# Parskatt/RoMa

Hardware: AMD Instinct MI355X
Metric: image-pairs/sec, roma_outdoor 560->864, batch=8 per GPU (higher is better)
Workload: dtype bf16; 1 GPU; roma_outdoor match() 560->864, symmetric, upsample_preds, 8 pairs/GPU/step, seeded synthetic weights + N(0,1) images; precision policy of the reference's bf16 timing script: bfloat16 DINOv2 + float16 autocast for VGG / decoder / refiners (ROMA_MIXED), f32 accumulate; precision_policy=mixed, global_batch=8, streams_per_gpu=2, parallelism=single GPU, outputs_finite=True

## Files before the change

roma_amd/csrc/elementwise.h:

```cpp
#pragma once
#include "common.h"

namespace roma {

int layernorm_launch(const float* x, const float* w, const float* b, void* out, long M, int D, float eps,
                     int dt_out, hipStream_t s);
int layernorm_launch_dt(const void* x, int dt_in, const float* w, const float* b, void* out, long M, int D, float eps,
                        int dt_out, hipStream_t s);

int conv3x3_c3_launch(const float* img, const float* w, const float* bias, void* out, int B, int H, int W,
                      int dt_out, hipStream_t s);

int im2col3x3_c3_launch(const float* img, void* out, int B, int H, int W, int dt_out, hipStream_t s);

int maxpool2x2_launch(const void* in, void* out, int B, int H, int W, int C, int dt, hipStream_t s);

int im2col_patch14_launch(const float* img, void* out, int B, int H, int W, int Kpad, int dt_out, hipStream_t s);

int assemble_tokens_launch(const float* patch, const float* cls, const float* pos, float* tokens, int B, int T,
                           int D, hipStream_t s);

int copy2d_launch(const void* in, long ldi, int dt_in, void* out, long ldo, int dt_out, long rows, int cols,
                  hipStream_t s);

int convert_from_bf16_launch(const void* in, void* out, long n, hipStream_t s);

int rownorm_launch(const void* in, long ld, int dt, float* norms, long M, int C, hipStream_t s);

int gp_basis_launch(const float* w, const float* b, float* Ft, int Dg, int h, int wdt, int npad, hipStream_t s, int copies = 1,
                    long stride = 0);

int transpose_launch(const float* in, float* out, int n, long ld, int batch, hipStream_t s, long stride_in = 0, long stride_out = 0);

int chol_diag_launch(float* A, long ld, long strideA, float* Linv, float* LinvT, int k, int nblk, int batch,
                     hipStream_t s);

int chol_col_launch(float* A, long ld, long strideA, float* LT, long strideLT, int n, int d, float* Linv, float* LinvT, int k,
                    int nblk, int batch, unsigned epoch, int use_leader, hipStream_t s);
int chol_col_restore_launch(float* A, long ld, long strideA, const float* LT, long strideLT, int n, int batch, hipStream_t s);

int pad_identity_launch(float* A, long ld, long strideA, int n, int npad, int batch, hipStream_t s);

int cls_to_flow_launch(const float* logits, long ld, float* flow, float* cert, long M, hipStream_t s);

struct RefinerInputArgs {
  const void* feat = nullptr;
  long ldf = 0;
  const float* flow = nullptr;
  void* d = nullptr;
  long ldd = 0;
  const float* emb_w = nullptr;
  const float* emb_b = nullptr;
  int B = 0, H = 0, W = 0, C = 0, E = 0, Kcorr = 0, nimg = 0, shift = 0;
  float disp_scale = 1.f;
  int dt = 0;
};
int refiner_input_launch(const RefinerInputArgs& a, hipStream_t s);

int dwconv5x5_launch(const void* in, void* out, const float* w, const float* bias, int B, int H, int W, int Cp,
                     int dt, hipStream_t s);
int dwconv5x5_ring_try_launch(const void* in, void* out, const float* w, const float* bias, int B, int H, int W, int Cp, int dt,
                              hipStream_t s);
// ... 23 lines not shown
```

roma_amd/csrc/gp.h:

```cpp
#pragma once
#include "arena.h"
#include "common.h"

namespace roma {

int gp_posterior(const void* pf, long ldf, int act_dt, int B, bool symmetric, int th, int tw, const float* gp_w,
                 const float* gp_b, float* mu, long ld_mu, Arena& arena, hipStream_t st, bool dry);

int cholesky_solve_t(float* A, float* Rt, float* LT, float* Linv, float* LinvT, int n, int d, int batch, hipStream_t st,
                     long strideA = 0, long strideR = 0);

}
```

roma_amd/csrc/gp.hip:

```cpp
#include "gp.h"

#include <atomic>

#include "dry_run.h"
#include "elementwise.h"
#include "gemm.h"
#include "tuning.h"

namespace roma {

int cholesky_solve_t(float* A, float* Rt, float* LT, float* Linv, float* LinvT, int n, int d, int batch, hipStream_t st,
                     long strideA, long strideR) {
  ROMA_REQUIRE(n % 64 == 0 && n > 0 && d % 4 == 0, "cholesky_solve: n must be a multiple of 64, d of 4");
  const int nblk = n / 64;
  const long sA = strideA > 0 ? strideA : (long)n * n, sR = strideR > 0 ? strideR : (long)d * n, sL = (long)nblk * 4096;
  const long sLT = (long)n * n;
  const bool aug_env = tuning(SW_GP_AUG) != 0;
  const bool aug = aug_env && Rt == A + (long)n * n && (batch == 1 || (sA == sR && sA >= (long)(n + d) * n));
  const int extra = aug ? d : 0;
  const bool col = aug && tuning(SW_GP_COL) != 0 && d >= 64 && d % 64 == 0;
  static std::atomic<unsigned> solve_epoch{0};
  const unsigned epoch = col ? ++solve_epoch : 0u;
  const int col_leader = col ? (int)tuning(SW_GP_COL_LEADER) : 0;
  for (int k = 0; k < nblk && col; ++k)
    if (int rc = chol_col_launch(A, n, sA, LT, sLT, n, d, Linv, LinvT, k, nblk, batch, epoch, col_leader, st)) return rc;
  if (col)
    if (int rc = chol_col_restore_launch(A, n, sA, LT, sLT, n, batch, st)) return rc;
  for (int k = 0; k < nblk && !col; ++k) {
    if (int rc = chol_diag_launch(A, n, sA, Linv, LinvT, k, nblk, batch, st)) return rc;
    const int mrem = n - (k + 1) * 64;
    if (mrem + extra <= 0) break;
    GemmArgs g;
    g.A = A + (long)(k + 1) * 64 * n + k * 64; g.lda = n; g.sA = sA;
    g.W = Linv + (long)k * 4096; g.ldw = 64; g.sW = sL;
    g.C = const_cast<float*>(static_cast<const float*>(g.A)); g.ldc = n; g.sC = sA;
// ... 18 lines not shown
    g.W = Linv + (long)k * 4096; g.ldw = 64; g.sW = sL;
    g.C = Rt + k * 64; g.ldc = n; g.sC = sR;
    g.M = d; g.N = 64; g.K = 64; g.batch = batch;
    if (int rc = gemm_launch(g, st)) return rc;
    const int mrem = n - (k + 1) * 64;
    if (mrem <= 0) break;
    GemmArgs u;
    u.A = Rt + k * 64; u.lda = n; u.sA = sR;
    u.W = A + (long)(k + 1) * 64 * n + k * 64; u.ldw = n; u.sW = sA;
    u.C = Rt + (k + 1) * 64; u.ldc = n; u.sC = sR;
    u.res = Rt + (k + 1) * 64; u.ldr = n; u.sR = sR;
    u.alpha = -1.f;
    u.M = d; u.N = mrem; u.K = 64; u.batch = batch;
    if (int rc = gemm_launch(u, st)) return rc;
  }
  const bool bwd_env = tuning(SW_GP_BWD2) != 0;
  if (bwd_env && nblk > 1) {
    GemmArgs m;
    m.A = LT; m.lda = n; m.sA = sLT; m.sA2 = 64;
    m.W = Linv; m.ldw = 64; m.sW = sL; m.sW2 = 4096;
    m.C = LT; m.ldc = n; m.sC = sLT; m.sC2 = 64;
    m.M = n; m.N = 64; m.K = 64; m.batch = batch; m.batch2 = nblk;
    if (int rc = gemm_launch(m, st)) return rc;
    for (int k = nblk - 1; k >= 1; --k) {
      GemmArgs u;
      u.A = Rt + k * 64; u.lda = n; u.sA = sR;
      u.W = LT + k * 64; u.ldw = n; u.sW = sLT;
      u.C = Rt; u.ldc = n; u.sC = sR;
      u.res = Rt; u.ldr = n; u.sR = sR;
      u.alpha = -1.f;
      u.M = d; u.N = k * 64; u.K = 64; u.batch = batch;
      if (int rc = gemm_launch(u, st)) return rc;
    }
    GemmArgs x;
    x.A = Rt; x.lda = n; x.sA = sR; x.sA2 = 64;
    x.W = LinvT; x.ldw = 64; x.sW = sL; x.sW2 = 4096;
    x.C = Rt; x.ldc = n; x.sC = sR; x.sC2 = 64;
    x.M = d; x.N = 64; x.K = 64; x.batch = batch; x.batch2 = nblk;
    return gemm_launch(x, st);
  }
  for (int k = nblk - 1; k >= 0; --k) {
    GemmArgs g;
    g.A = Rt + k * 64; g.lda = n; g.sA = sR;
    g.W = LinvT + (long)k * 4096; g.ldw = 64; g.sW = sL;
    g.C = Rt + k * 64; g.ldc = n; g.sC = sR;
    g.M = d; g.N = 64; g.K = 64; g.batch = batch;
    if (int rc = gemm_launch(g, st)) return rc;
// ... 5 lines not shown
    u.res = Rt; u.ldr = n; u.sR = sR;
    u.alpha = -1.f;
    u.M = d; u.N = k * 64; u.K = 64; u.batch = batch;
    if (int rc = gemm_launch(u, st)) return rc;
  }
  return 0;
}

int gp_posterior(const void* pf, long ldf, int act_dt, int B, bool symmetric, int th, int tw, const float* gp_w,
                 const float* gp_b, float* mu, long ld_mu, Arena& arena, hipStream_t st, bool dry) {
  const size_t esz = act_dt == DT_F32 ? 4 : 2;
  const int nimg = 2 * B, ndp = symmetric ? 2 * B : B, shift = B;
  const int n = th * tw, npad = (int)round_up(n, 64), nblk = npad / 64;
  auto AL = [&](size_t elems, size_t es) { return arena.alloc(elems * es); };
  auto off = [&](const void* p, long elems) -> const void* { return static_cast<const char*>(p) + elems * (long)esz; };
  float* norms = (float*)AL((size_t)nimg * n, 4);
  const long saug = (long)(npad + 512) * npad;
  float* Kyy = (float*)AL((size_t)nimg * saug, 4);
  float* Rt = Kyy + (long)npad * npad;
  float* LT = (float*)AL((size_t)nimg * npad * npad, 4);
  float* Kxy = (float*)AL((size_t)ndp * n * npad, 4);
  float* Linv = (float*)AL((size_t)nimg * nblk * 4096, 4);
  float* LinvT = (float*)AL((size_t)nimg * nblk * 4096, 4);
  if (!dry && arena.overflow) return -5;
  RUN(rownorm_launch(pf, ldf, act_dt, norms, (long)nimg * n, 512, st));
  const int j0 = symmetric ? 0 : B, nj = symmetric ? nimg : B;
  {
    GemmArgs g;
    g.A = off(pf, (long)j0 * n * ldf); g.lda = ldf; g.sA = (long)n * ldf;
    g.W = g.A; g.ldw = ldf; g.sW = g.sA;
    g.C = Kyy + (long)j0 * saug; g.ldc = npad; g.sC = saug;
    g.M = n; g.N = n; g.K = 512; g.batch = nj; g.in_dt = act_dt; g.out_dt = DT_F32; g.mode = EPI_COSK;
    g.nx = norms + (long)j0 * n; g.ny = g.nx; g.sNx = n; g.sNy = n; g.inv_t = 1.0f / 0.2f; g.diag_add = 0.1f;
    RUN(gemm_launch(g, st));
  }
  RUN(pad_identity_launch(Kyy + (long)j0 * saug, npad, saug, n, npad, nj, st));
  if (!dry && npad != n) ROMA_CHECK_HIP(hipMemsetAsync(Kxy, 0, (size_t)ndp * n * npad * 4, st));
  for (int half = 0; half < (symmetric ? 2 : 1); ++half) {
    GemmArgs g;
    const int i0 = half * B, s0 = (i0 + shift) % nimg;
    g.A = off(pf, (long)i0 * n * ldf); g.lda = ldf; g.sA = (long)n * ldf;
    g.W = off(pf, (long)s0 * n * ldf); g.ldw = ldf; g.sW = (long)n * ldf;
    g.C = Kxy + (long)i0 * n * npad; g.ldc = npad; g.sC = (long)n * npad;
    g.M = n; g.N = n; g.K = 512; g.batch = B; g.in_dt = act_dt; g.out_dt = DT_F32; g.mode = EPI_COSK;
    g.nx = norms + (long)i0 * n; g.ny = norms + (long)s0 * n; g.sNx = n; g.sNy = n; g.inv_t = 1.0f / 0.2f;
    RUN(gemm_launch(g, st));
  }
  RUN(gp_basis_launch(gp_w, gp_b, Rt + (long)j0 * saug, 512, th, tw, npad, st, nj, saug));
  RUN(cholesky_solve_t(Kyy + (long)j0 * saug, Rt + (long)j0 * saug, LT + (long)j0 * npad * npad,
                          Linv + (long)j0 * nblk * 4096, LinvT + (long)j0 * nblk * 4096, npad, 512, nj, st, saug, saug));
  for (int half = 0; half < (symmetric ? 2 : 1); ++half) {
    GemmArgs g;
    const int i0 = half * B, s0 = (i0 + shift) % nimg;
    g.A = Kxy + (long)i0 * n * npad; g.lda = npad; g.sA = (long)n * npad;
    g.W = Rt + (long)s0 * saug; g.ldw = npad; g.sW = saug;
    g.C = mu + (long)i0 * n * ld_mu; g.ldc = ld_mu; g.sC = (long)n * ld_mu;
    g.M = n; g.N = 512; g.K = npad; g.batch = B;
    RUN(gemm_launch(g, st));
  }
  return 0;
}
}
```

roma_amd/csrc/local_corr.h:

```cpp
#pragma once
#include "common.h"

namespace roma {

struct LocalCorrArgs {
  const void* f0 = nullptr;
  const void* f1 = nullptr;
  const float* warp = nullptr;
  void* out = nullptr;
  int B = 0, H = 0, W = 0, C = 0;
  int radius = 0;
  int K = 0;
  long ld0 = 0, ld1 = 0, ldo = 0;
  int nimg = 0, f1_shift = 0;
  float scale = 1.f;
  int in_dt = 0, out_dt = 0;
  int nearest = 0;
  int* ws = nullptr;
  long ws_bytes = 0;
  int force_gather = 0;
  int pxmax = 0;
  int bin_ts = 0, bin_nx = 0, bin_ny = 0, ws_bins = 0, ws_qlist = 0;
  int sort_bands = 0;
  long ws_tclass = 0, ws_hist = 0;
};

long local_corr_ws_ints(int B, int H, int W, int radius);

int local_corr_window_launch(const LocalCorrArgs& a, hipStream_t stream);
int local_corr_general_launch(const LocalCorrArgs& a, hipStream_t stream);

}
```

roma_amd/csrc/local_corr.hip:

```cpp
#include "local_corr.h"
#include "tuning.h"
#include <stdio.h>
#include <stdlib.h>
#include <algorithm>
#include "gemm.h"

namespace roma {

template <typename T> struct LcIO;
template <> struct LcIO<float> {
  static constexpr int CE = 4;
  __device__ static inline void ld(const float* p, float* v) {
    f32x4 x = *reinterpret_cast<const f32x4*>(p);
    v[0] = x[0]; v[1] = x[1]; v[2] = x[2]; v[3] = x[3];
  }
};
template <> struct LcIO<bf16_t> {
  static constexpr int CE = 8;
  __device__ static inline void ld(const bf16_t* p, float* v) {
    uint4 u = *reinterpret_cast<const uint4*>(p);
    v[0] = h16_lo(u.x); v[1] = h16_hi(u.x);
    v[2] = h16_lo(u.y); v[3] = h16_hi(u.y);
    v[4] = h16_lo(u.z); v[5] = h16_hi(u.z);
    v[6] = h16_lo(u.w); v[7] = h16_hi(u.w);
// ... 157 lines not shown

template <int R, typename T, typename TOUT, bool MFMA, bool LIST = false>
__global__ __launch_bounds__((LcGeom<R, MFMA>::NTHR), 2) void local_corr_tile_kernel(const LocalCorrArgs a) {
  constexpr int P = 2 * R + 2, KW = 2 * R + 1, K = KW * KW;
  constexpr int NTHR = LcGeom<R, MFMA>::NTHR, NWV = NTHR / 64, NBG = NWV / 2;
  constexpr int NR = (P + NWV - 1) / NWV;
  constexpr int NBW = MFMA ? ((LcGeom<R, MFMA>::PXMAX + 31) / 32 + NBG - 1) / NBG : 1;
  static_assert(!MFMA || sizeof(T) == 2, "the MFMA form takes 16-bit features");
  constexpr int CC = LcDot<T>::CC;
  constexpr int LC_STAGE = LcGeom<R, MFMA>::STAGE, LC_PXMAX = LcGeom<R, MFMA>::PXMAX, NPRE = LcGeom<R, MFMA>::NPRE;
  extern __shared__ __attribute__((aligned(16))) char lds[];
  int* qx0 = reinterpret_cast<int*>(lds + LC_STAGE);
  int* qy0 = qx0 + 64;
  float* qfx = reinterpret_cast<float*>(qy0 + 64);
  float* qfy = qfx + 64;
  int* tinfo = reinterpret_cast<int*>(qfy + 64);
  int* qpx = tinfo + 8;

  const int tid = threadIdx.x, lane = tid & 63, wave = tid >> 6;
  const int tiles_x = (a.W + LC_TQ - 1) / LC_TQ, tiles_y = (a.H + LC_TQ - 1) / LC_TQ;
  const int tpi = tiles_x * tiles_y;
  const long HW = (long)a.H * a.W;
  const int* tlist = a.ws + 4 + a.B * tpi;
  for (int tidx = blockIdx.x; tidx < (LIST ? a.ws[2] : a.ws[1]); tidx += gridDim.x) {
  __syncthreads();
  int b, qin;
  if constexpr (LIST) {
    const int* ql = a.ws + a.ws_qlist + (long)tidx * 64;
    const int g = ql[lane];
    b = __shfl(g, 0) / (int)HW;
    qin = g >= 0 ? g - b * (int)HW : -1;
  } else {
    const int tile = tlist[tidx];
    b = tile / tpi;
    const int trem = tile - b * tpi;
    const int ty = trem / tiles_x, tx = trem - ty * tiles_x;
    const int qy = ty * LC_TQ + (lane >> 3), qx = tx * LC_TQ + (lane & 7);
    qin = (qy < a.H && qx < a.W) ? qy * a.W + qx : -1;
  }

  const bool qvalid = qin >= 0;
  const long qpix = (long)b * HW + (qvalid ? qin : 0);
  int x0 = 0, y0 = 0;
  float fx = 0.f, fy = 0.f;
  if (qvalid) {
    unnormalize_floor(a.warp[qpix * 2 + 0], a.W, x0, fx);
    unnormalize_floor(a.warp[qpix * 2 + 1], a.H, y0, fy);
  }
// ... 498 lines not shown
}
long local_corr_ws_ints(int B, int H, int W, int radius) {
  if (radius != 2 && radius != 3 && radius != 7) return 0;
  const long tiles = (long)B * ((H + LC_TQ - 1) / LC_TQ) * ((W + LC_TQ - 1) / LC_TQ);
  const int ts = lc_bin_ts(radius), P = 2 * radius + 2;
  const long nbins = (long)B * ((W + P) / ts + 1) * ((H + P) / ts + 1);
  return 4 + 2 * tiles + 3 * nbins + 64 * (tiles + nbins) + tiles + lc_sort_bands(B, (H + LC_TQ - 1) / LC_TQ) * nbins;
}

template <int R, typename T, typename TOUT, bool MFMA>
static int launch_tiled(const LocalCorrArgs& a0, hipStream_t stream) {
  LocalCorrArgs a = a0;
  const int tiles = a.B * ((a.H + LC_TQ - 1) / LC_TQ) * ((a.W + LC_TQ - 1) / LC_TQ);
  constexpr int P = 2 * R + 2;
  a.bin_ts = lc_bin_ts(R);
  a.bin_nx = (a.W + P) / a.bin_ts + 1;
  a.bin_ny = (a.H + P) / a.bin_ts + 1;
  const long nbins = (long)a.B * a.bin_nx * a.bin_ny;
  a.ws_bins = 4 + 2 * tiles;
  a.ws_qlist = a.ws_bins + 3 * (int)nbins;
  const int lc_bin = tuning(SW_LC_BIN);
  const bool binned = lc_bin != 0 && (long)a.B * a.H * a.W < (1l << 31) &&
                      (a.bin_ts + P - 1) * (a.bin_ts + P - 1) <= LcGeom<R, MFMA>::PXMAX;
  const bool lds_sort = binned && lc_bin == 1 && a.bin_nx * a.bin_ny <= LC_SORT_MAXBINS && 64 * ((long)tiles + nbins) < (1l << 31);
  a.ws_tclass = a.ws_qlist + 64 * ((long)tiles + nbins);
  a.ws_hist = a.ws_tclass + tiles;
  a.sort_bands = lds_sort ? lc_sort_bands(a.B, (a.H + LC_TQ - 1) / LC_TQ) : 0;
  const size_t need = (size_t)local_corr_ws_ints(a.B, a.H, a.W, R) * sizeof(int);
  bool own_ws = false;
  if (!a.ws) {
    ROMA_CHECK_HIP(hipMallocAsync(reinterpret_cast<void**>(&a.ws), need, stream));
    own_ws = true;
  } else {
    ROMA_REQUIRE((size_t)a.ws_bytes >= need, "local_corr(window): work-list scratch too small");
  }
  a.force_gather = tuning_override(SW_LC_MODE) == 1 ? 1 : 0;
  ROMA_CHECK_HIP(hipMemsetAsync(a.ws, 0, 4 * sizeof(int), stream));
  const size_t lds_tile = (size_t)LcGeom<R, MFMA>::STAGE + 5 * 64 * 4 + 32;
  a.pxmax = LcGeom<R, MFMA>::PXMAX;
  static bool attr_set[64] = {false};
  int dev = 0;
  ROMA_CHECK_HIP(hipGetDevice(&dev));
  if (dev < 0 || dev >= 64 || !attr_set[dev]) {
    ROMA_CHECK_HIP(hipFuncSetAttribute(reinterpret_cast<const void*>(&local_corr_tile_kernel<R, T, TOUT, MFMA>),
                                       hipFuncAttributeMaxDynamicSharedMemorySize, (int)lds_tile));
    if (dev >= 0 && dev < 64) attr_set[dev] = true;
  }
// ... 6 lines not shown
      const dim3 sgrid((unsigned)a.sort_bands, (unsigned)a.B);
      hipLaunchKernelGGL((local_corr_sort_kernel<R, false>), sgrid, dim3(LC_SORT_NTHR), 0, stream, a);
      ROMA_LAUNCH_CHECK();
      hipLaunchKernelGGL(local_corr_bin_scan_kernel, dim3(1), dim3(1024), 0, stream, a);
      ROMA_LAUNCH_CHECK();
      hipLaunchKernelGGL((local_corr_sort_kernel<R, true>), sgrid, dim3(LC_SORT_NTHR), 0, stream, a);
      ROMA_LAUNCH_CHECK();
    } else {
      ROMA_CHECK_HIP(hipMemsetAsync(a.ws + a.ws_bins, 0, (size_t)3 * nbins * sizeof(int), stream));
      ROMA_CHECK_HIP(hipMemsetAsync(a.ws + a.ws_qlist, 0xff, (size_t)64 * (tiles + nbins) * sizeof(int), stream));
      hipLaunchKernelGGL((local_corr_bin_kernel<R, false>), dim3((unsigned)tiles), dim3(64), 0, stream, a);
      ROMA_LAUNCH_CHECK();
      hipLaunchKernelGGL(local_corr_bin_scan_kernel, dim3(1), dim3(1024), 0, stream, a);
      ROMA_LAUNCH_CHECK();
      hipLaunchKernelGGL((local_corr_bin_kernel<R, true>), dim3((unsigned)tiles), dim3(64), 0, stream, a);
      ROMA_LAUNCH_CHECK();
    }
    static bool attr_set_l[64] = {false};
    if (dev < 0 || dev >= 64 || !attr_set_l[dev]) {
      ROMA_CHECK_HIP(hipFuncSetAttribute(reinterpret_cast<const void*>(&local_corr_tile_kernel<R, T, TOUT, MFMA, true>),
                                         hipFuncAttributeMaxDynamicSharedMemorySize, (int)lds_tile));
      if (dev >= 0 && dev < 64) attr_set_l[dev] = true;
    }
    const long max_items = (long)tiles + nbins;
    hipLaunchKernelGGL((local_corr_tile_kernel<R, T, TOUT, MFMA, true>), dim3((unsigned)std::min<long>(max_items, 8192)), dim3(LcGeom<R, MFMA>::NTHR),
                       lds_tile, stream, a);
    ROMA_LAUNCH_CHECK();
  } else {
    hipLaunchKernelGGL((local_corr_list_kernel<R, T, TOUT, 4>), dim3((unsigned)tiles * 16u), dim3(256), (size_t)4 * a.C * sizeof(float),
                       stream, a);
    ROMA_LAUNCH_CHECK();
  }
  if (own_ws) ROMA_CHECK_HIP(hipFreeAsync(a.ws, stream));
  return 0;
}

template <int R>
static int launch_window_r(const LocalCorrArgs& a, hipStream_t stream) {
  const long total = (long)a.B * a.H * a.W;
  dim3 grid((unsigned)((total + 3) / 4));
  size_t lds = (size_t)4 * a.C * sizeof(float);
  const double es_in = a.in_dt == DT_F32 ? 4.0 : 2.0, es_out = a.out_dt == DT_F32 ? 4.0 : 2.0;
  char pname[64];
  snprintf(pname, sizeof pname, "local_corr_window_kernel<%d,%s>", R, a.in_dt == DT_F32 ? "f32" : ROMA_H16_NAME);
  ProfScope ps(pname, (double)total * (2.0 * a.C * es_in + 8.0 + (2.0 * R + 1) * (2.0 * R + 1) * es_out), "byte", stream);
  const int mode = tuning(SW_LC_MODE);
  const int cc = a.in_dt == DT_F32 ? 32 : 64;
// ... 55 lines not shown
```

roma_amd/csrc/refiner_input.hip:

```cpp
#include <algorithm>
#include <stdio.h>
#include "elementwise_device.h"
#include "tuning.h"

namespace roma {

__device__ __forceinline__ void bilinear_taps(float wx, float wy, int W, int H, int& x0, int& y0, float (&wgt)[4]) {
  float ix = ((wx + 1.f) * W - 1.f) * 0.5f, iy = ((wy + 1.f) * H - 1.f) * 0.5f;
  ix = fminf(fmaxf(ix, -1.0e6f), 1.0e6f);
  iy = fminf(fmaxf(iy, -1.0e6f), 1.0e6f);
  const float fx0 = floorf(ix), fy0 = floorf(iy);
  x0 = (int)fx0; y0 = (int)fy0;
  const float tx = ix - fx0, ty = iy - fy0;
  wgt[0] = (1.f - tx) * (1.f - ty); wgt[1] = tx * (1.f - ty); wgt[2] = (1.f - tx) * ty; wgt[3] = tx * ty;
}

template <typename T>
__global__ __launch_bounds__(256) void refiner_input_kernel(const RefinerInputArgs a) {
  const int lane = threadIdx.x & 63;
  const long HW = (long)a.H * a.W;
  const long pix = (long)blockIdx.x * 4 + (threadIdx.x >> 6);
  if (pix >= (long)a.B * HW) return;
  const int b = (int)(pix / HW);
  const long p = pix - (long)b * HW;
// ... 57 lines not shown
      float wgt[4];
      bilinear_taps(wx, wy, a.W, a.H, x0, y0, wgt);
      float acc = 0.f;
#pragma unroll
      for (int t = 0; t < 4; ++t) {
        const int yy = y0 + (t >> 1), xx = x0 + (t & 1);
        if (yy >= 0 && yy < a.H && xx >= 0 && xx < a.W)
          acc += wgt[t] * ElemIO<T>::ld(fs + ((long)yy * a.W + xx) * a.ldf + cc);
      }
      ElemIO<T>::st(d + c, acc);
    } else if (c < 2 * a.C + a.E) {
      const int e = c - 2 * a.C;
      const int y = (int)(p / a.W), x = (int)(p - (long)y * a.W);
      const float dx = a.disp_scale * (a.flow[pix * 2 + 0] - pix_coord(x, a.W));
      const float dy = a.disp_scale * (a.flow[pix * 2 + 1] - pix_coord(y, a.H));
      ElemIO<T>::st(d + c, a.emb_w[e * 2 + 0] * dx + a.emb_w[e * 2 + 1] * dy + a.emb_b[e]);
    } else if (c >= 2 * a.C + a.E + a.Kcorr) {
      ElemIO<T>::st(d + c, 0.f);
    }
  }
}

template <typename T, int C, int E>
__global__ __launch_bounds__(256) void refiner_input_pix_kernel(const RefinerInputArgs a) {
  constexpr int LDF = 16, LDD = 24;
  const long HW = (long)a.H * a.W;
  const long pix = (long)blockIdx.x * 256 + threadIdx.x;
  if (pix >= (long)a.B * HW) return;
  const int b = (int)(pix / HW);
  const long p = pix - (long)b * HW;
  const int y = (int)(p / a.W), x = (int)(p - (long)y * a.W);
  const T* feat = reinterpret_cast<const T*>(a.feat);
  const T* fq = feat + ((long)b * HW + p) * LDF;
  const int simg = (b + a.shift) % a.nimg;
  const T* fs = feat + (long)simg * HW * LDF;
  if constexpr (sizeof(T) == 2) {
    static_assert(C <= 16 && 2 * C + E <= LDD && LDD == 24 && LDF == 16, "layout");
    float q[16], xh[16];
    VecIO<T>::ld(fq, q);
    VecIO<T>::ld(fq + 8, q + 8);
#pragma unroll
    for (int j = 0; j < 16; ++j) xh[j] = 0.f;
    const float wx = a.flow[pix * 2 + 0], wy = a.flow[pix * 2 + 1];
    int x0, y0;
    float wgt[4];
    bilinear_taps(wx, wy, a.W, a.H, x0, y0, wgt);
#pragma unroll
    for (int t = 0; t < 4; ++t) {
      const int yy = y0 + (t >> 1), xx = x0 + (t & 1);
      if (yy >= 0 && yy < a.H && xx >= 0 && xx < a.W) {
        const T* r = fs + ((long)yy * a.W + xx) * LDF;
        float v[16];
        VecIO<T>::ld(r, v);
        VecIO<T>::ld(r + 8, v + 8);
#pragma unroll
        for (int j = 0; j < C; ++j) xh[j] += wgt[t] * v[j];
      }
    }
    const float dx = a.disp_scale * (wx - pix_coord(x, a.W)), dy = a.disp_scale * (wy - pix_coord(y, a.H));
    float o[LDD];
#pragma unroll
    for (int c = 0; c < C; ++c) {
      o[c] = q[c];
      o[C + c] = xh[c];
    }
#pragma unroll
    for (int e = 0; e < E; ++e) o[2 * C + e] = a.emb_w[e * 2 + 0] * dx + a.emb_w[e * 2 + 1] * dy + a.emb_b[e];
#pragma unroll
    for (int c = 2 * C + E; c < LDD; ++c) o[c] = 0.f;
    T* d = reinterpret_cast<T*>(a.d) + pix * LDD;
#pragma unroll
    for (int c8 = 0; c8 < LDD / 8; ++c8) VecIO<T>::st(d + c8 * 8, o + c8 * 8);
    return;
  }
  float q[12], xh[12];
#pragma unroll
  for (int c4 = 0; c4 < 3; ++c4) {
    const f32x4 v = ElemIO<T>::ld4(fq + c4 * 4);
#pragma unroll
    for (int j = 0; j < 4; ++j) {
      q[c4 * 4 + j] = v[j];
      xh[c4 * 4 + j] = 0.f;
    }
  }
  const float wx = a.flow[pix * 2 + 0], wy = a.flow[pix * 2 + 1];
  int x0, y0;
  float wgt[4];
  bilinear_taps(wx, wy, a.W, a.H, x0, y0, wgt);
#pragma unroll
  for (int t = 0; t < 4; ++t) {
    const int yy = y0 + (t >> 1), xx = x0 + (t & 1);
    if (yy >= 0 && yy < a.H && xx >= 0 && xx < a.W) {
// ... 60 lines not shown
      float tv[CV];
      VecIO<T>::ld(fs + off[t] + c, tv);
#pragma unroll
      for (int j = 0; j < CV; ++j) r[j] = ok[t] ? r[j] + wgt[t] * tv[j] : r[j];
    }
    VecIO<T>::st(d + a.C + c, r);
  }
  const float dx = a.disp_scale * (wx - pix_coord(x, a.W)), dy = a.disp_scale * (wy - pix_coord(y, a.H));
  for (int e = sub; e < a.E; e += lpp) {
    const float v = a.emb_w[e * 2 + 0] * dx + a.emb_w[e * 2 + 1] * dy + a.emb_b[e];
    ElemIO<T>::st(d + 2 * a.C + e, v);
  }
  for (long c = 2 * a.C + a.E + a.Kcorr + sub; c < a.ldd; c += lpp) ElemIO<T>::st(d + c, 0.f);
}

int refiner_input_launch(const RefinerInputArgs& a, hipStream_t s) {
  const long npix = (long)a.B * a.H * a.W;
  const double es = a.dt == DT_F32 ? 4.0 : 2.0;
  char pname[64];
  snprintf(pname, sizeof pname, "refiner_input_warp<C=%d,%s>", a.C, a.dt == DT_F32 ? "f32" : ROMA_H16_NAME);
  ProfScope ps(pname, (double)npix * (2.0 * a.C * es + 8.0 + (double)(a.ldd - a.Kcorr) * es), "byte", s);
  if (a.C == 9 && a.E == 6 && a.Kcorr == 0 && a.ldf == 16 && a.ldd == 24) {
    dim3 grid((unsigned)((npix + 255) / 256));
    ROMA_DT_SWITCH(a.dt, T, hipLaunchKernelGGL((refiner_input_pix_kernel<T, 9, 6>), grid, dim3(256), 0, s, a));
    ROMA_LAUNCH_CHECK();
    return 0;
  }
  if (a.C % 4 != 0 || a.C < 32) {
    const long total = npix * a.ldd;
    dim3 grid((unsigned)std::min<long>((total + 255) / 256, 1 << 20));
    ROMA_DT_SWITCH(a.dt, T, hipLaunchKernelGGL(refiner_input_small_kernel<T>, grid, dim3(256), 0, s, a));
    ROMA_LAUNCH_CHECK();
    return 0;
  }
  ROMA_REQUIRE(a.ldf % 4 == 0 && a.ldd % 4 == 0, "refiner_input: strides must be multiples of 4");
  {
    const int cv = a.dt == DT_F32 ? 4 : 8;
    const bool aligned = ((reinterpret_cast<uintptr_t>(a.feat) | reinterpret_cast<uintptr_t>(a.d)) & 15) == 0;
    const bool vec_off = tuning(SW_RI_VEC) == 0;
    if (!vec_off && aligned && a.C % cv == 0 && a.ldf % cv == 0 && a.ldd % cv == 0) {
      int lpp = 1;
      while (lpp < 64 && lpp * cv < a.C) lpp *= 2;
      const long per_wg = 4 * (64 / lpp);
      dim3 vgrid((unsigned)((npix + per_wg - 1) / per_wg));
      ROMA_DT_SWITCH(a.dt, T, hipLaunchKernelGGL(refiner_input_vec_kernel<T>, vgrid, dim3(256), 0, s, a, lpp));
      ROMA_LAUNCH_CHECK();
// ... 11 lines not shown
```

roma_amd/csrc/tuning.hip:

```cpp
#include "tuning.h"

#include <stdlib.h>
#include <string.h>

#include "../../include/roma_hip.h"

namespace roma {
void set_error(const std::string& msg);
namespace {

struct Row {
  Switch id;
  const char* key;
  const char* env;
  long def;
  int floor;
  const char* doc;
};

constexpr Row ROWS[] = {
    {SW_GEMM8P, "gemm8p", "ROMA_GEMM8P", 1, 0, "large bf16 GEMMs on the 8-phase 256 x 256 kernel (1) or on the one-barrier-per-slab kernel (0)"},
    {SW_GEMM_DBG, "gemm_dbg", "ROMA_GEMM_DBG", 0, 0, "experiment bits of the GEMM kernels (1 skip output stores, 2 skip the K loop, 2048 no streaming stores, ...)"},
    {SW_GEMM8P_WALK, "gemm8p_walk", nullptr, -1, 1, "gemm8p: tile rows per group of the persistent walk (1 = row major); unset = 8 from 24 tile columns on, else 1"},
    {SW_GEMM8P_SCHED, "gemm8p_sched", "ROMA_GEMM8P_SCHED", 1, 0, "gemm8p K-loop schedule: 1 k-half phases, 0 quadrant phases (tools builds only)"},
    {SW_GEMM8P_MAXWG, "gemm8p_maxwg", nullptr, -1, 8, "gemm8p, measurement only: cap the persistent grid at n workgroups (a multiple of 8); unset = one per CU"},
    {SW_WS1X1, "ws1x1", "ROMA_WS1X1", 1, 0, "N = K = 576 refiner 1x1 on the weight-stationary kernel (1) or on the 256 x 192 tile kernel (0)"},
    {SW_LC_MODE, "lc_mode", "ROMA_LC_MODE", 0, 0, "local correlation: 0 tiled form + gather work list, 1 every tile on the gather list (key only), 2 per-pixel kernel"},
    {SW_LC_BIN, "lc_bin", "ROMA_LC_BIN", 1, 0, "local correlation: queries of incoherent tiles sorted by target bin, counters in LDS (1) or device atomics (2), or gathered per query (0)"},
    {SW_CONV64, "conv64", "ROMA_CONV64", 7, 0, "weight-stationary VGG front end, bit mask: 1 the Cin = 64 kernels, 2 the Cin = 128 kernel, 4 the fused first layer"},
    {SW_CONV_PATCH, "conv_patch", "ROMA_CONV_PATCH", 1, 0, "patch-resident 3x3 kernel for slab-major VGG layers (1) or gemm8p (0); environment 0 also packs tap-major weights"},
    {SW_ATTN_XCD, "attn_xcd", "ROMA_ATTN_XCD", 1, 0, "attention work items in per-XCD bands of (batch, head) (1) or in plain order (0)"},
    {SW_ATTN_EXP2, "attn_exp2", nullptr, -1, 0, "tools only: force the 2^x softmax of the 16-bit attention kernel on / off; unset = as the caller says"},
    {SW_DW_RING, "dw_ring", "ROMA_DW_RING", 1, 0, "depthwise 5x5: 0 register-prefetch kernel, 1 ring kernel for the large launches, 2 ring kernel for every shape it takes"},
    {SW_GP_COL, "gp_col", "ROMA_GP_COL", 1, 0, "GP Cholesky left-looking, one launch per block column (1) or the right-looking launch chain (0)"},
    {SW_POOL_PROJ, "pool_proj", "ROMA_POOL_PROJ", 1, 0, "max-pool + proj head of strides 1 / 2 in one pass (1) or as separate kernels (0)"},
    {SW_GP_COL_LEADER, "gp_col_leader", "ROMA_GP_COL_LEADER", 1, 0, "block-column Cholesky: a leader workgroup factorises the diagonal block, its product formed one launch ahead (1) or in its own launch (2), or every workgroup its own copy (0)"},
    {SW_GEMM8P_MINM, nullptr, "ROMA_GEMM8P_MINM", 2048, 0, "gemm8p: smallest M it takes for the wide (N >= 2048) dense launches"},
    {SW_GEMM_NT, nullptr, "ROMA_GEMM_NT", 1, 0, "non-temporal output stores in the 16-bit GEMM row writer"},
    {SW_GEMM_F32_FILL, nullptr, "ROMA_GEMM_F32_FILL", 1, 0, "exact-f32 GEMMs below 192 tiles of 256 x 256 run on 128 x 128 tiles"},
    {SW_GEMM_SMALLM, nullptr, "ROMA_GEMM_SMALLM", 1, 0, "GEMMs below 320 tiles of 128 x 128 run on 128 x 64 tiles"},
    {SW_CONV64_SY, nullptr, "ROMA_CONV64_SY", 0, 0, "conv64 strip height in rows; 0 = the split of H with the fewest rounds"},
    {SW_CONV_KORDER, nullptr, "ROMA_CONV_KORDER", 1, 0, "VGG layers with Cout >= 256 pack slab-major weight rows (read when a handle is created)"},
    {SW_RB_SY, nullptr, "ROMA_RB_SY", 0, 0, "fused refiner block strip height in rows; 0 = the split of H with the fewest rounds"},
    {SW_DWR_MAXSY, nullptr, "ROMA_DWR_MAXSY", 1 << 20, 0, "depthwise ring kernel: cap of the strip height in rows (at least 6)"},
    {SW_DW_RING_MINELEMS, nullptr, "ROMA_DW_RING_MINELEMS", 64l << 20, 0, "dw_ring = 1: smallest launch, in elements, that goes to the ring kernel"},
    {SW_RI_VEC, nullptr, "ROMA_RI_VEC", 1, 0, "refiner_input on the 16-byte vector kernel where alignment allows"},
    {SW_OUT_ROW, nullptr, "ROMA_OUT_ROW", 1, 0, "refiner_out: row kernel for C = 24 in 16-bit storage"},
    {SW_OUT_LPR, nullptr, "ROMA_OUT_LPR", 1, 0, "refiner_out, 16-bit: lanes per row chosen to fill the 16-byte pieces best"},
    {SW_OUT_ROWS_IT, nullptr, "ROMA_OUT_ROWS_IT", 0, 0, "refiner_out: row groups per wave (even, >= 2); otherwise 8"},
    {SW_GP_AUG, nullptr, "ROMA_GP_AUG", 1, 0, "GP Cholesky: right-hand sides stored behind A ride along the factorisation (0 = separate forward loop)"},
    {SW_GP_BWD2, nullptr, "ROMA_GP_BWD2", 1, 0, "GP Cholesky: backward substitution with one launch per step (0 = two)"},
    {SW_COMPOSE_OUT, nullptr, "ROMA_COMPOSE_OUT", 1, 0, "initial value of the handle option compose_out_conv (read when a handle is created)"},
    {SW_VIT_RES_F32, nullptr, "ROMA_VIT_RES_F32", 0, 0, "force DINOv2's f32 residual stream in the 16-bit modes"},
    {SW_STREAMS, nullptr, "ROMA_STREAMS", 0, 0, "number of sub-batch streams of match(); 0 = the handle's option"},
    {SW_STREAMS_SERIAL, nullptr, "ROMA_STREAMS_SERIAL", 0, 0, "diagnostic: sub-batch streams run one after the other"},
    {SW_DEBUG_DUAL_SLOT, nullptr, "ROMA_DEBUG_DUAL_SLOT", -1, 0, "diagnostic: keep the stream split in debug mode, sub-batch k captures the stages of ROMA_DEBUG_ONLY"},
};
constexpr int NROWS = sizeof(ROWS) / sizeof(ROWS[0]);
constexpr bool rows_in_enum_order() {
  for (int i = 0; i < NROWS; ++i)
    if (ROWS[i].id != i) return false;
  return true;
}
static_assert(NROWS == SW_COUNT && rows_in_enum_order(), "one row per Switch, in enum order");
constexpr bool json_plain(const char* s) {
  for (; s && *s; ++s)
    if (*s == '"' || *s == '\\' || *s < ' ') return false;
  return true;
}
// ... 59 lines not shown
```

Before: 109.8 image-pairs/s.

## Batch GP backward substitution, band local-corr items per XCD, coalesce refiner input

Adds a fused backward-substitution kernel for the GP Cholesky solve that processes up to four block columns per launch, keeping intermediate results in LDS and a side buffer instead of issuing one GEMM launch per block column. Separately, the local-correlation sorted work list is now walked in interleaved bands (per-XCD grouping), and the 16-bit refiner-input kernel stages whole rows through LDS so global loads and stores are fully coalesced. The aim is fewer launches and better cache locality and memory coalescing, at the cost of extra kernel complexity and a workspace buffer.

```diff
diff --git a/roma_amd/csrc/chol_bwd.hip b/roma_amd/csrc/chol_bwd.hip
--- /dev/null
+++ b/roma_amd/csrc/chol_bwd.hip
@@ -0,0 +1,152 @@
+#include <algorithm>
+
+#include "elementwise.h"
+
+namespace roma {
+
+namespace {
+
+constexpr int CB_MAXG = 4;
+constexpr int CB_SLOT = 64 * 256;
+constexpr int CB_STAGE = 4096;
+constexpr int CB_LDSB = (CB_MAXG - 1) * 64;
+
+__global__ __launch_bounds__(256) void chol_col_bwd_kernel(float* R, long sR, const float* __restrict__ LT, long sLT, int n, int k,
+                                                           int gg, int nd, float* SB, long sSB, int pk, int pn) {
+  extern __shared__ __attribute__((aligned(16))) char lds[];
+  const int tid = threadIdx.x, lane = tid & 63;
+  const int wave = __builtin_amdgcn_readfirstlane(tid >> 6);
+  const int wm = wave >> 1, wn = wave & 1;
+  const int l31 = lane & 31, h = lane >> 5;
+  float* Rb = R + (long)blockIdx.z * sR + (long)blockIdx.y * 64 * n;
+  const float* LTb = LT + (long)blockIdx.z * sLT;
+  float* SBb = SB + (long)blockIdx.z * sSB + (long)blockIdx.y * 64 * CB_LDSB;
+  const bool writer = blockIdx.x == 0;
+
+  if (writer) {
+    for (int i = tid; i < pn * 1024; i += 256) {
+      const int q = i >> 10, row = (i >> 4) & 63, ch = i & 15;
+      *reinterpret_cast<f32x4*>(Rb + (long)row * n + (pk - 1 - q) * 64 + ch * 4) =
+          *reinterpret_cast<const f32x4*>(SBb + (long)row * CB_LDSB + q * 64 + ch * 4);
+    }
+  }
+  if (gg == 0) return;
+
+  for (int i = tid; i < 1024; i += 256) {
+    const int row = i >> 4, ch = i & 15;
+    *reinterpret_cast<f32x4*>(lds + row * 256 + ((ch ^ (row & 15)) << 4)) = *reinterpret_cast<const f32x4*>(Rb + (long)row * n + k * 64 + ch * 4);
+  }
+  __syncthreads();
+
+  char* stage = lds + gg * CB_SLOT + wave * CB_STAGE;
+  const int nfull = k - gg + 1;
+  const int j0 = blockIdx.x * nd;
+  const int ndm = min(nd, nfull - j0);
+  const int ntg = gg - 1 + ndm;
+  const auto load_w = [&](f32x4 (&w)[8], int ks, int t) {
+    const float* p = LTb + (long)(t * 64 + 32 * wn + l31) * n + ks * 64 + 4 * h;
+#pragma unroll
+    for (int i = 0; i < 8; ++i) w[i] = *reinterpret_cast<const f32x4*>(p + 8 * i);
+  };
+  const auto target_block = [&](int q) { return q < gg - 1 ? k - 1 - q : j0 + q - (gg - 1); };
+  const int prow = 32 * wm + (lane >> 3), pcol = 32 * wn + 4 * (lane & 7);
+
+  f32x4 wcur[8], wnext[8];
+  load_w(wcur, k, target_block(0));
+  for (int q = 0; q < ntg; ++q) {
+    const int t = target_block(q);
+    const int nst = q < gg - 1 ? q + 1 : gg;
+    f32x4 val[4];
+#pragma unroll
+    for (int i = 0; i < 4; ++i) val[i] = *reinterpret_cast<const f32x4*>(Rb + (long)(prow + 8 * i) * n + t * 64 + pcol);
+    for (int u = 0; u < nst; ++u) {
+      const bool more = u + 1 < nst || q + 1 < ntg;
+      if (u + 1 < nst) load_w(wnext, k - u - 1, t);
+      else if (q + 1 < ntg) load_w(wnext, k, target_block(q + 1));
+      const char* crow = lds + u * CB_SLOT + (32 * wm + l31) * 256;
+      f32x4 av[8];
+#pragma unroll
+      for (int i = 0; i < 8; ++i) av[i] = *reinterpret_cast<const f32x4*>(crow + (((2 * i + h) ^ (l31 & 15)) << 4));
+      f32x16 acc;
+#pragma unroll
+      for (int e = 0; e < 16; ++e) acc[e] = 0.f;
+#pragma unroll
+      for (int i = 0; i < 8; ++i)
+#pragma unroll
+        for (int c = 0; c < 4; ++c) acc = __builtin_amdgcn_mfma_f32_32x32x2f32(wcur[i][c], av[i][c], acc, 0, 0, 0);
+#pragma unroll
+      for (int rg = 0; rg < 4; ++rg)
+        *reinterpret_cast<f32x4*>(stage + l31 * 128 + (((2 * rg + h) ^ (l31 & 7)) << 4)) =
+            f32x4{acc[4 * rg], acc[4 * rg + 1], acc[4 * rg + 2], acc[4 * rg + 3]};
+      __builtin_amdgcn_wave_barrier();
+#pragma unroll
+      for (int i = 0; i < 4; ++i) {
+        const int row = (lane >> 3) + 8 * i;
+        const f32x4 v = *reinterpret_cast<const f32x4*>(stage + row * 128 + (((lane & 7) ^ (row & 7)) << 4));
+#pragma unroll
+        for (int j = 0; j < 4; ++j) val[i][j] = val[i][j] - v[j];
+      }
+      __builtin_amdgcn_wave_barrier();
+#pragma unroll
+      for (int i = 0; i < 8; ++i) wcur[i] = more ? wnext[i] : wcur[i];
+    }
+    if (q < gg - 1) {
+#pragma unroll
+      for (int i = 0; i < 4; ++i) {
+        const int row = prow + 8 * i;
+        *reinterpret_cast<f32x4*>(lds + (q + 1) * CB_SLOT + row * 256 + (((pcol >> 2) ^ (row & 15)) << 4)) = val[i];
+        if (writer) *reinterpret_cast<f32x4*>(SBb + (long)row * CB_LDSB + q * 64 + pcol) = val[i];
+      }
+      __syncthreads();
+    } else {
+#pragma unroll
+      for (int i = 0; i < 4; ++i) *reinterpret_cast<f32x4*>(Rb + (long)(prow + 8 * i) * n + t * 64 + pcol) = val[i];
+    }
+  }
+}
+
+int cb_pick_nd(int nfull, int row_tiles, int batch, int gg) {
+  int best = 1;
+  long best_cost = -1;
+  for (int nd = 1; nd <= 4; ++nd) {
+    const long wgs = (long)((nfull + nd - 1) / nd) * row_tiles * batch;
+    const long cost = ((wgs + 511) / 512) * (gg * (gg - 1) / 2 + gg * std::min(nd, nfull));
+    if (best_cost < 0 || cost < best_cost) {
+      best_cost = cost;
+      best = nd;
+    }
+  }
+  return best;
+}
+
+}
+
+long chol_bwd_ws_floats(int d, int batch) { return (long)batch * d * CB_LDSB; }
+
+int chol_bwd_launch(float* R, long strideR, const float* LT, long strideLT, int n, int d, int k, int gg, float* ws, int pk, int pn,
+                    int batch, hipStream_t s) {
+  ROMA_REQUIRE(n % 64 == 0 && d % 64 == 0 && d >= 64 && gg >= 0 && gg <= CB_MAXG && gg <= k && pn >= 0 && pn < CB_MAXG && ws,
+               "chol_bwd: n, d multiples of 64, at most 4 steps per launch, a side buffer");
+  ROMA_REQUIRE(((reinterpret_cast<uintptr_t>(R) | reinterpret_cast<uintptr_t>(LT) | reinterpret_cast<uintptr_t>(ws)) & 15) == 0 &&
+               strideR % 4 == 0 && strideLT % 4 == 0, "chol_bwd: buffers must be 16-byte aligned");
+  const int row_tiles = d / 64;
+  const int nfull = k - gg + 1;
+  const int nd = gg > 0 ? cb_pick_nd(nfull, row_tiles, batch, gg) : 1;
+  const unsigned gx = gg > 0 ? (unsigned)((nfull + nd - 1) / nd) : 1u;
+  const size_t lds = gg > 0 ? (size_t)gg * CB_SLOT + 4 * CB_STAGE : 0;
+  static bool attr_set[64] = {false};
+  int dev = 0;
+  ROMA_CHECK_HIP(hipGetDevice(&dev));
+  if (dev < 0 || dev >= 64 || !attr_set[dev]) {
+    ROMA_CHECK_HIP(hipFuncSetAttribute(reinterpret_cast<const void*>(&chol_col_bwd_kernel), hipFuncAttributeMaxDynamicSharedMemorySize,
+                                       CB_MAXG * CB_SLOT + 4 * CB_STAGE));
+    if (dev >= 0 && dev < 64) attr_set[dev] = true;
+  }
+  ProfScope ps("chol_col_bwd_kernel", 2.0 * d * 64.0 * 64.0 * batch * (gg * (double)nfull + gg * (gg - 1) / 2), "flop", s);
+  hipLaunchKernelGGL(chol_col_bwd_kernel, dim3(gx, (unsigned)row_tiles, (unsigned)batch), dim3(256), lds, s, R, strideR, LT, strideLT, n,
+                     k, gg, nd, ws, (long)d * CB_LDSB, pk, pn);
+  ROMA_LAUNCH_CHECK();
+  return 0;
+}
+
+}
diff --git a/roma_amd/csrc/elementwise.h b/roma_amd/csrc/elementwise.h
--- a/roma_amd/csrc/elementwise.h
+++ b/roma_amd/csrc/elementwise.h
@@ -38,6 +38,10 @@
 int chol_col_launch(float* A, long ld, long strideA, float* LT, long strideLT, int n, int d, float* Linv, float* LinvT, int k,
                     int nblk, int batch, unsigned epoch, int use_leader, hipStream_t s);
 int chol_col_restore_launch(float* A, long ld, long strideA, const float* LT, long strideLT, int n, int batch, hipStream_t s);
+
+long chol_bwd_ws_floats(int d, int batch);
+int chol_bwd_launch(float* R, long strideR, const float* LT, long strideLT, int n, int d, int k, int gg, float* ws, int pk, int pn,
+                    int batch, hipStream_t s);
 
 int pad_identity_launch(float* A, long ld, long strideA, int n, int npad, int batch, hipStream_t s);
 
diff --git a/roma_amd/csrc/gp.h b/roma_amd/csrc/gp.h
--- a/roma_amd/csrc/gp.h
+++ b/roma_amd/csrc/gp.h
@@ -8,6 +8,6 @@
                  const float* gp_b, float* mu, long ld_mu, Arena& arena, hipStream_t st, bool dry);
 
 int cholesky_solve_t(float* A, float* Rt, float* LT, float* Linv, float* LinvT, int n, int d, int batch, hipStream_t st,
-                     long strideA = 0, long strideR = 0);
+                     long strideA = 0, long strideR = 0, float* bwd_ws = nullptr);
 
 }
diff --git a/roma_amd/csrc/gp.hip b/roma_amd/csrc/gp.hip
--- a/roma_amd/csrc/gp.hip
+++ b/roma_amd/csrc/gp.hip
@@ -1,5 +1,6 @@
 #include "gp.h"
 
+#include <algorithm>
 #include <atomic>
 
 #include "dry_run.h"
@@ -10,7 +11,7 @@
 namespace roma {
 
 int cholesky_solve_t(float* A, float* Rt, float* LT, float* Linv, float* LinvT, int n, int d, int batch, hipStream_t st,
-                     long strideA, long strideR) {
+                     long strideA, long strideR, float* bwd_ws) {
   ROMA_REQUIRE(n % 64 == 0 && n > 0 && d % 4 == 0, "cholesky_solve: n must be a multiple of 64, d of 4");
   const int nblk = n / 64;
   const long sA = strideA > 0 ? strideA : (long)n * n, sR = strideR > 0 ? strideR : (long)d * n, sL = (long)nblk * 4096;
@@ -75,7 +76,23 @@
     m.C = LT; m.ldc = n; m.sC = sLT; m.sC2 = 64;
     m.M = n; m.N = 64; m.K = 64; m.batch = batch; m.batch2 = nblk;
     if (int rc = gemm_launch(m, st)) return rc;
-    for (int k = nblk - 1; k >= 1; --k) {
+    const long gpc = tuning(SW_GP_COL);
+    const int bwd_cols = d % 64 != 0 || gpc == 0 || gpc == 3 ? 1 : (gpc == 2 ? 2 : 4);
+    if (bwd_cols > 1) {
+      float* ws = bwd_ws;
+      if (!ws) ROMA_CHECK_HIP(hipMallocAsync(reinterpret_cast<void**>(&ws), (size_t)chol_bwd_ws_floats(d, batch) * sizeof(float), st));
+      int rc = 0, pk = 0, pn = 0;
+      for (int k = nblk - 1; k >= 1 && !rc;) {
+        const int gg = std::min(bwd_cols, k);
+        rc = chol_bwd_launch(Rt, sR, LT, sLT, n, d, k, gg, ws, pk, pn, batch, st);
+        pk = k; pn = gg - 1;
+        k -= gg;
+      }
+      if (!rc && pn > 0) rc = chol_bwd_launch(Rt, sR, LT, sLT, n, d, 0, 0, ws, pk, pn, batch, st);
+      if (!bwd_ws) ROMA_CHECK_HIP(hipFreeAsync(ws, st));
+      if (rc) return rc;
+    }
+    for (int k = nblk - 1; k >= 1 && bwd_cols == 1; --k) {
       GemmArgs u;
       u.A = Rt + k * 64; u.lda = n; u.sA = sR;
       u.W = LT + k * 64; u.ldw = n; u.sW = sLT;
@@ -127,6 +144,7 @@
   float* Kxy = (float*)AL((size_t)ndp * n * npad, 4);
   float* Linv = (float*)AL((size_t)nimg * nblk * 4096, 4);
   float* LinvT = (float*)AL((size_t)nimg * nblk * 4096, 4);
+  float* bwd_ws = (float*)AL((size_t)chol_bwd_ws_floats(512, nimg), 4);
   if (!dry && arena.overflow) return -5;
   RUN(rownorm_launch(pf, ldf, act_dt, norms, (long)nimg * n, 512, st));
   const int j0 = symmetric ? 0 : B, nj = symmetric ? nimg : B;
@@ -153,7 +171,7 @@
   }
   RUN(gp_basis_launch(gp_w, gp_b, Rt + (long)j0 * saug, 512, th, tw, npad, st, nj, saug));
   RUN(cholesky_solve_t(Kyy + (long)j0 * saug, Rt + (long)j0 * saug, LT + (long)j0 * npad * npad,
-                          Linv + (long)j0 * nblk * 4096, LinvT + (long)j0 * nblk * 4096, npad, 512, nj, st, saug, saug));
+                          Linv + (long)j0 * nblk * 4096, LinvT + (long)j0 * nblk * 4096, npad, 512, nj, st, saug, saug, bwd_ws));
   for (int half = 0; half < (symmetric ? 2 : 1); ++half) {
     GemmArgs g;
     const int i0 = half * B, s0 = (i0 + shift) % nimg;
diff --git a/roma_amd/csrc/local_corr.h b/roma_amd/csrc/local_corr.h
--- a/roma_amd/csrc/local_corr.h
+++ b/roma_amd/csrc/local_corr.h
@@ -23,6 +23,7 @@
   int bin_ts = 0, bin_nx = 0, bin_ny = 0, ws_bins = 0, ws_qlist = 0;
   int sort_bands = 0;
   long ws_tclass = 0, ws_hist = 0;
+  int item_bands = 0;
 };
 
 long local_corr_ws_ints(int B, int H, int W, int radius);
diff --git a/roma_amd/csrc/local_corr.hip b/roma_amd/csrc/local_corr.hip
--- a/roma_amd/csrc/local_corr.hip
+++ b/roma_amd/csrc/local_corr.hip
@@ -203,8 +203,16 @@
   const int tpi = tiles_x * tiles_y;
   const long HW = (long)a.H * a.W;
   const int* tlist = a.ws + 4 + a.B * tpi;
-  for (int tidx = blockIdx.x; tidx < (LIST ? a.ws[2] : a.ws[1]); tidx += gridDim.x) {
+  const int nitems = LIST ? a.ws[2] : a.ws[1];
+  const bool bands = LIST && a.item_bands;
+  const int per = (nitems + 7) >> 3;
+  for (int v = blockIdx.x; v < (bands ? 8 * per : nitems); v += gridDim.x) {
   __syncthreads();
+  int tidx = v;
+  if (bands) {
+    tidx = (v & 7) * per + (v >> 3);
+    if (tidx >= nitems) continue;
+  }
   int b, qin;
   if constexpr (LIST) {
     const int* ql = a.ws + a.ws_qlist + (long)tidx * 64;
@@ -749,7 +757,9 @@
   const int lc_bin = tuning(SW_LC_BIN);
   const bool binned = lc_bin != 0 && (long)a.B * a.H * a.W < (1l << 31) &&
                       (a.bin_ts + P - 1) * (a.bin_ts + P - 1) <= LcGeom<R, MFMA>::PXMAX;
-  const bool lds_sort = binned && lc_bin == 1 && a.bin_nx * a.bin_ny <= LC_SORT_MAXBINS && 64 * ((long)tiles + nbins) < (1l << 31);
+  const bool lds_sort = binned && (lc_bin == 1 || lc_bin == 3) && a.bin_nx * a.bin_ny <= LC_SORT_MAXBINS &&
+                        64 * ((long)tiles + nbins) < (1l << 31);
+  a.item_bands = lc_bin != 3;
   a.ws_tclass = a.ws_qlist + 64 * ((long)tiles + nbins);
   a.ws_hist = a.ws_tclass + tiles;
   a.sort_bands = lds_sort ? lc_sort_bands(a.B, (a.H + LC_TQ - 1) / LC_TQ) : 0;
@@ -802,7 +812,7 @@
                                          hipFuncAttributeMaxDynamicSharedMemorySize, (int)lds_tile));
       if (dev >= 0 && dev < 64) attr_set_l[dev] = true;
     }
-    const long max_items = (long)tiles + nbins;
+    const long max_items = round_up((long)tiles + nbins, 8);
     hipLaunchKernelGGL((local_corr_tile_kernel<R, T, TOUT, MFMA, true>), dim3((unsigned)std::min<long>(max_items, 8192)), dim3(LcGeom<R, MFMA>::NTHR),
                        lds_tile, stream, a);
     ROMA_LAUNCH_CHECK();
diff --git a/roma_amd/csrc/refiner_input.hip b/roma_amd/csrc/refiner_input.hip
--- a/roma_amd/csrc/refiner_input.hip
+++ b/roma_amd/csrc/refiner_input.hip
@@ -103,6 +103,92 @@
 }
 
 template <typename T, int C, int E>
+__device__ __forceinline__ void refiner_input_pix16(const RefinerInputArgs& a, long pix, const float (&q)[16], float (&o)[24]) {
+  constexpr int LDF = 16, LDD = 24;
+  static_assert(sizeof(T) == 2 && C <= 16 && 2 * C + E <= LDD, "layout");
+  const long HW = (long)a.H * a.W;
+  const int b = (int)(pix / HW);
+  const long p = pix - (long)b * HW;
+  const int y = (int)(p / a.W), x = (int)(p - (long)y * a.W);
+  const int simg = (b + a.shift) % a.nimg;
+  const T* fs = reinterpret_cast<const T*>(a.feat) + (long)simg * HW * LDF;
+  float xh[16];
+#pragma unroll
+  for (int j = 0; j < 16; ++j) xh[j] = 0.f;
+  const float wx = a.flow[pix * 2 + 0], wy = a.flow[pix * 2 + 1];
+  int x0, y0;
+  float wgt[4];
+  bilinear_taps(wx, wy, a.W, a.H, x0, y0, wgt);
+#pragma unroll
+  for (int t = 0; t < 4; ++t) {
+    const int yy = y0 + (t >> 1), xx = x0 + (t & 1);
+    if (yy >= 0 && yy < a.H && xx >= 0 && xx < a.W) {
+      const T* r = fs + ((long)yy * a.W + xx) * LDF;
+      float v[16];
+      VecIO<T>::ld(r, v);
+      VecIO<T>::ld(r + 8, v + 8);
+#pragma unroll
+      for (int j = 0; j < C; ++j) xh[j] += wgt[t] * v[j];
+    }
+  }
+  const float dx = a.disp_scale * (wx - pix_coord(x, a.W)), dy = a.disp_scale * (wy - pix_coord(y, a.H));
+#pragma unroll
+  for (int c = 0; c < C; ++c) {
+    o[c] = q[c];
+    o[C + c] = xh[c];
+  }
+#pragma unroll
+  for (int e = 0; e < E; ++e) o[2 * C + e] = a.emb_w[e * 2 + 0] * dx + a.emb_w[e * 2 + 1] * dy + a.emb_b[e];
+#pragma unroll
+  for (int c = 2 * C + E; c < LDD; ++c) o[c] = 0.f;
+}
+
+template <typename T, int C, int E>
+__global__ __launch_bounds__(256) void refiner_input_pix_rows_kernel(const RefinerInputArgs a) {
+  constexpr int LDF = 16, LDD = 24;
+  __shared__ __attribute__((aligned(16))) uint4 slab_all[4][3 * 64];
+  const int lane = threadIdx.x & 63;
+  uint4* slab = slab_all[threadIdx.x >> 6];
+  const long total = (long)a.B * a.H * a.W;
+  const long pix0 = (long)blockIdx.x * 256 + (threadIdx.x & ~63);
+  if (pix0 >= total) return;
+  const int np = total - pix0 < 64 ? (int)(total - pix0) : 64;
+  const uint4* fq = reinterpret_cast<const uint4*>(reinterpret_cast<const T*>(a.feat) + pix0 * LDF);
+  uint4* d = reinterpret_cast<uint4*>(reinterpret_cast<T*>(a.d) + pix0 * LDD);
+#pragma unroll
+  for (int k = 0; k < 2; ++k) {
+    const int piece = lane + 64 * k;
+    if (piece < 2 * np) slab[piece] = fq[piece];
+  }
+  __builtin_amdgcn_wave_barrier();
+  uint4 u[3];
+  if (lane < np) {
+    float q[16], o[LDD];
+    VecIO<T>::cvt(slab[2 * lane], q);
+    VecIO<T>::cvt(slab[2 * lane + 1], q + 8);
+    refiner_input_pix16<T, C, E>(a, pix0 + lane, q, o);
+#pragma unroll
+    for (int c8 = 0; c8 < 3; ++c8) {
+      u[c8].x = pack_bf16x2(o[c8 * 8 + 0], o[c8 * 8 + 1]);
+      u[c8].y = pack_bf16x2(o[c8 * 8 + 2], o[c8 * 8 + 3]);
+      u[c8].z = pack_bf16x2(o[c8 * 8 + 4], o[c8 * 8 + 5]);
+      u[c8].w = pack_bf16x2(o[c8 * 8 + 6], o[c8 * 8 + 7]);
+    }
+  }
+  __builtin_amdgcn_wave_barrier();
+  if (lane < np) {
+#pragma unroll
+    for (int c8 = 0; c8 < 3; ++c8) slab[3 * lane + c8] = u[c8];
+  }
+  __builtin_amdgcn_wave_barrier();
+#pragma unroll
+  for (int k = 0; k < 3; ++k) {
+    const int piece = lane + 64 * k;
+    if (piece < 3 * np) d[piece] = slab[piece];
+  }
+}
+
+template <typename T, int C, int E>
 __global__ __launch_bounds__(256) void refiner_input_pix_kernel(const RefinerInputArgs a) {
   constexpr int LDF = 16, LDD = 24;
   const long HW = (long)a.H * a.W;
@@ -116,39 +202,11 @@
   const int simg = (b + a.shift) % a.nimg;
   const T* fs = feat + (long)simg * HW * LDF;
   if constexpr (sizeof(T) == 2) {
-    static_assert(C <= 16 && 2 * C + E <= LDD && LDD == 24 && LDF == 16, "layout");
-    float q[16], xh[16];
+    static_assert(LDD == 24 && LDF == 16, "layout");
+    float q[16], o[LDD];
     VecIO<T>::ld(fq, q);
     VecIO<T>::ld(fq + 8, q + 8);
-#pragma unroll
-    for (int j = 0; j < 16; ++j) xh[j] = 0.f;
-    const float wx = a.flow[pix * 2 + 0], wy = a.flow[pix * 2 + 1];
-    int x0, y0;
-    float wgt[4];
-    bilinear_taps(wx, wy, a.W, a.H, x0, y0, wgt);
-#pragma unroll
-    for (int t = 0; t < 4; ++t) {
-      const int yy = y0 + (t >> 1), xx = x0 + (t & 1);
-      if (yy >= 0 && yy < a.H && xx >= 0 && xx < a.W) {
-        const T* r = fs + ((long)yy * a.W + xx) * LDF;
-        float v[16];
-        VecIO<T>::ld(r, v);
-        VecIO<T>::ld(r + 8, v + 8);
-#pragma unroll
-        for (int j = 0; j < C; ++j) xh[j] += wgt[t] * v[j];
-      }
-    }
-    const float dx = a.disp_scale * (wx - pix_coord(x, a.W)), dy = a.disp_scale * (wy - pix_coord(y, a.H));
-    float o[LDD];
-#pragma unroll
-    for (int c = 0; c < C; ++c) {
-      o[c] = q[c];
-      o[C + c] = xh[c];
-    }
-#pragma unroll
-    for (int e = 0; e < E; ++e) o[2 * C + e] = a.emb_w[e * 2 + 0] * dx + a.emb_w[e * 2 + 1] * dy + a.emb_b[e];
-#pragma unroll
-    for (int c = 2 * C + E; c < LDD; ++c) o[c] = 0.f;
+    refiner_input_pix16<T, C, E>(a, pix, q, o);
     T* d = reinterpret_cast<T*>(a.d) + pix * LDD;
 #pragma unroll
     for (int c8 = 0; c8 < LDD / 8; ++c8) VecIO<T>::st(d + c8 * 8, o + c8 * 8);
@@ -255,6 +313,12 @@
   ProfScope ps(pname, (double)npix * (2.0 * a.C * es + 8.0 + (double)(a.ldd - a.Kcorr) * es), "byte", s);
   if (a.C == 9 && a.E == 6 && a.Kcorr == 0 && a.ldf == 16 && a.ldd == 24) {
     dim3 grid((unsigned)((npix + 255) / 256));
+    const bool aligned = ((reinterpret_cast<uintptr_t>(a.feat) | reinterpret_cast<uintptr_t>(a.d)) & 15) == 0;
+    if (a.dt != DT_F32 && aligned && tuning(SW_RI_VEC) == 1) {
+      hipLaunchKernelGGL((refiner_input_pix_rows_kernel<bf16_t, 9, 6>), grid, dim3(256), 0, s, a);
+      ROMA_LAUNCH_CHECK();
+      return 0;
+    }
     ROMA_DT_SWITCH(a.dt, T, hipLaunchKernelGGL((refiner_input_pix_kernel<T, 9, 6>), grid, dim3(256), 0, s, a));
     ROMA_LAUNCH_CHECK();
     return 0;
diff --git a/roma_amd/csrc/tuning.hip b/roma_amd/csrc/tuning.hip
--- a/roma_amd/csrc/tuning.hip
+++ b/roma_amd/csrc/tuning.hip
@@ -26,13 +26,13 @@
     {SW_GEMM8P_MAXWG, "gemm8p_maxwg", nullptr, -1, 8, "gemm8p, measurement only: cap the persistent grid at n workgroups (a multiple of 8); unset = one per CU"},
     {SW_WS1X1, "ws1x1", "ROMA_WS1X1", 1, 0, "N = K = 576 refiner 1x1 on the weight-stationary kernel (1) or on the 256 x 192 tile kernel (0)"},
     {SW_LC_MODE, "lc_mode", "ROMA_LC_MODE", 0, 0, "local correlation: 0 tiled form + gather work list, 1 every tile on the gather list (key only), 2 per-pixel kernel"},
-    {SW_LC_BIN, "lc_bin", "ROMA_LC_BIN", 1, 0, "local correlation: queries of incoherent tiles sorted by target bin, counters in LDS (1) or device atomics (2), or gathered per query (0)"},
+    {SW_LC_BIN, "lc_bin", "ROMA_LC_BIN", 1, 0, "local correlation: queries of incoherent tiles sorted by target bin, counters in LDS (1) or device atomics (2), or gathered per query (0); 3 = as 1 with the sorted items in plain order, not in per-XCD bands"},
     {SW_CONV64, "conv64", "ROMA_CONV64", 7, 0, "weight-stationary VGG front end, bit mask: 1 the Cin = 64 kernels, 2 the Cin = 128 kernel, 4 the fused first layer"},
     {SW_CONV_PATCH, "conv_patch", "ROMA_CONV_PATCH", 1, 0, "patch-resident 3x3 kernel for slab-major VGG layers (1) or gemm8p (0); environment 0 also packs tap-major weights"},
     {SW_ATTN_XCD, "attn_xcd", "ROMA_ATTN_XCD", 1, 0, "attention work items in per-XCD bands of (batch, head) (1) or in plain order (0)"},
     {SW_ATTN_EXP2, "attn_exp2", nullptr, -1, 0, "tools only: force the 2^x softmax of the 16-bit attention kernel on / off; unset = as the caller says"},
     {SW_DW_RING, "dw_ring", "ROMA_DW_RING", 1, 0, "depthwise 5x5: 0 register-prefetch kernel, 1 ring kernel for the large launches, 2 ring kernel for every shape it takes"},
-    {SW_GP_COL, "gp_col", "ROMA_GP_COL", 1, 0, "GP Cholesky left-looking, one launch per block column (1) or the right-looking launch chain (0)"},
+    {SW_GP_COL, "gp_col", "ROMA_GP_COL", 1, 0, "GP Cholesky left-looking, one launch per block column (1) or the right-looking launch chain (0); backward substitution four block columns per launch, 2 / 3 = as 1 with two / one per launch, 0 one"},
     {SW_POOL_PROJ, "pool_proj", "ROMA_POOL_PROJ", 1, 0, "max-pool + proj head of strides 1 / 2 in one pass (1) or as separate kernels (0)"},
     {SW_GP_COL_LEADER, "gp_col_leader", "ROMA_GP_COL_LEADER", 1, 0, "block-column Cholesky: a leader workgroup factorises the diagonal block, its product formed one launch ahead (1) or in its own launch (2), or every workgroup its own copy (0)"},
     {SW_GEMM8P_MINM, nullptr, "ROMA_GEMM8P_MINM", 2048, 0, "gemm8p: smallest M it takes for the wide (N >= 2048) dense launches"},
@@ -44,7 +44,7 @@
     {SW_RB_SY, nullptr, "ROMA_RB_SY", 0, 0, "fused refiner block strip height in rows; 0 = the split of H with the fewest rounds"},
     {SW_DWR_MAXSY, nullptr, "ROMA_DWR_MAXSY", 1 << 20, 0, "depthwise ring kernel: cap of the strip height in rows (at least 6)"},
     {SW_DW_RING_MINELEMS, nullptr, "ROMA_DW_RING_MINELEMS", 64l << 20, 0, "dw_ring = 1: smallest launch, in elements, that goes to the ring kernel"},
-    {SW_RI_VEC, nullptr, "ROMA_RI_VEC", 1, 0, "refiner_input on the 16-byte vector kernel where alignment allows"},
+    {SW_RI_VEC, nullptr, "ROMA_RI_VEC", 1, 0, "refiner_input on the 16-byte vector kernel where alignment allows; 1 = also the stride-1 kernel with whole-row memory instructions (16-bit), 2 = with per-pixel accesses"},
     {SW_OUT_ROW, nullptr, "ROMA_OUT_ROW", 1, 0, "refiner_out: row kernel for C = 24 in 16-bit storage"},
     {SW_OUT_LPR, nullptr, "ROMA_OUT_LPR", 1, 0, "refiner_out, 16-bit: lanes per row chosen to fill the 16-byte pieces best"},
     {SW_OUT_ROWS_IT, nullptr, "ROMA_OUT_ROWS_IT", 0, 0, "refiner_out: row groups per wave (even, >= 2); otherwise 8"},
```

After: 110.1 image-pairs/s, median of 6. About the same (+0.3%).
